# arangesh/TrackMPNN

Measured on AMD Instinct MI355X. Metric: graph_edges_per_sec_fwd_bwd, higher is better.
Workload: dtype f32; 1 GPU; C2 KITTI Car/RRC-shaped rolling windows: 7 frames, D_t~clip(Poisson(6),1,20), F=8 (2d), H=64, K=0, diff; 1 fwd per frame + 1 bwd per window; 16384 windows/GPU batched block-diagonally (64 distinct seeds tiled); windows_per_gpu=16384, rows_final=6762496, parallelism=sequence-dp1

## Files before the change

include/tmpnn.h:

```cpp
#ifndef TMPNN_H
#define TMPNN_H

#include <stddef.h>
#include <stdint.h>

#ifdef __cplusplus
extern "C" {
#endif

#define TMPNN_ABI_VERSION 4

#define TMPNN_OK 0
#define TMPNN_EINVAL (-1)
#define TMPNN_ELAUNCH (-2)
#define TMPNN_EWORKSPACE (-3)

typedef void* tmpnn_stream;
typedef void* tmpnn_event;

typedef struct tmpnn_seg_plan {
    int32_t T;
    int32_t I;
    int32_t nsplit;
    const int32_t* t_row;
// ... 111 lines not shown
                        float* d_msg, int ld_dmsg, float* d_h, int ld_dh,
                        const int32_t* add_src, const int32_t* add_dst, const float* add_msg, int ld_add,
                        float* dW_ih, float* dW_hh, float* db_ih, float* db_hh,
                        void* ws, size_t ws_bytes, tmpnn_stream stream);
int tmpnn_gru_bwd_fused_zero_state_available(int H, int IN, int xmode);
int tmpnn_gru_bwd_fused_zero_state(const int32_t* rows, int R, const int32_t* src, const int32_t* dst, int IN,
                                   const float* h, int ld_h, int H, const float* w_ih, const float* b_hn,
                                   const float* gates, size_t gate_plane, const float* d_hout, int ld_dhout,
                                   const float* dy, const float* w_head, float* d_msg, int ld_dmsg,
                                   float* dW_ih, float* db_ih, float* db_hh,
                                   void* ws, size_t ws_bytes, tmpnn_stream stream);

int tmpnn_gru_fwd_tiles(const tmpnn_edge_tiles* tiles, int R, const float* proj, int ld_proj, const float* h, int ld_h, int H,
                        const float* whh_t, const float* b_ih, const float* b_hh, float* h_out, int ld_out, float* gates,
                        size_t gate_plane, const float* w_head, float* logit_part, size_t part_stride, tmpnn_stream stream);

int tmpnn_rows_linear(const int32_t* rows, int R, const float* in, int ld_in, int H, const float* wt, int NOUT,
                      float* out, int ld_out, tmpnn_stream stream);

int tmpnn_transpose(const float* in, int rows, int cols, float* out, tmpnn_stream stream);

int tmpnn_input_bn_fwd(const float* xdet, int ld_x, int F, int nd, const int32_t* seg_ptr,
                       const int32_t* seg_cnt, const int32_t* seg_of_det ,
                       int S, int H, int training,
                       const float* w1, const float* b1, const float* gamma, const float* beta,
                       float* running_mean, float* running_var,
                       const float* w2, const float* b2,
                       float* y_save, float* mean, float* rstd, float* ws_a ,
                       const int32_t* out_row, float* h_new, int ld_h, tmpnn_stream stream);
size_t tmpnn_input_bn_bwd_ws(int nd, int S, int H, int F);
// ... 233 lines not shown
```

trackmpnn_amd/_lib.py:

```python
from __future__ import annotations

import ctypes as C

import torch
import os
import re
from typing import Dict, List, Optional

_HERE = os.path.dirname(os.path.abspath(__file__))
LIB_PATH = os.environ.get('TMPNN_LIB_PATH') or os.path.join(_HERE, 'lib', 'libtmpnn.so')
HEADER_PATH = os.path.join(os.path.dirname(_HERE), 'include', 'tmpnn.h')

ABI_VERSION = 4

c_int = C.c_int
c_void_p = C.c_void_p
c_size_t = C.c_size_t
c_float = C.c_float


class CSegPlan(C.Structure):
    _fields_ = [('T', C.c_int32), ('I', C.c_int32), ('nsplit', C.c_int32), ('t_row', c_void_p), ('items', c_void_p),
                ('rowptr2', c_void_p), ('inc2', c_void_p), ('ws', c_void_p), ('ws_floats', c_size_t)]

# ... 62 lines not shown
                              c_void_p, c_void_p, c_void_p, c_void_p, c_void_p, c_void_p, c_int, c_void_p]),
    'tmpnn_att_bwd_ws': (c_size_t, [c_int, c_int, c_int, c_int]),
    'tmpnn_att_index': (c_int, [_GP, c_void_p, c_void_p, c_void_p, c_void_p, c_void_p, c_void_p]),
    'tmpnn_att_bwd': (c_int, [_GP, c_void_p, c_void_p, c_void_p, c_int, c_int, c_int, c_void_p, c_void_p, c_void_p,
                              c_float, c_void_p, c_void_p, c_void_p, c_void_p, c_void_p, c_int, c_void_p, c_size_t,
                              c_void_p, c_int, c_void_p, c_void_p, c_void_p]),
    'tmpnn_att_bwd_heads': (c_int, [_GP, c_void_p, c_void_p, c_void_p, c_int, c_int, c_int, c_void_p, c_void_p,
                                    c_void_p, c_float, c_void_p, c_void_p, c_void_p, c_void_p, c_void_p, c_int, c_void_p,
                                    c_size_t, c_void_p, c_int, c_void_p, c_void_p, c_void_p]),
    'tmpnn_gru_fwd': (c_int, [c_void_p, c_int, c_int, c_void_p, c_void_p, c_void_p, c_int, c_int, c_int,
                              c_void_p, c_int, c_int, c_void_p, c_void_p, c_void_p, c_void_p,
                              c_void_p, c_int, c_void_p, c_size_t, c_void_p, c_void_p, c_size_t, c_void_p]),
    'tmpnn_gru_fwd_head_parts': (c_int, [c_int, c_int, c_int]),
    'tmpnn_gru_fwd_tiles': (c_int, [_TP, c_int, c_void_p, c_int, c_void_p, c_int, c_int, c_void_p, c_void_p, c_void_p,
                                    c_void_p, c_int, c_void_p, c_size_t, c_void_p, c_void_p, c_size_t, c_void_p]),
    'tmpnn_heads_finish': (c_int, [c_void_p, c_size_t, c_int, c_int, c_void_p, c_void_p, c_void_p, c_void_p, c_void_p, c_void_p]),
    'tmpnn_gru_bwd_data': (c_int, [c_void_p, c_int, c_int, c_void_p, c_int, c_int, c_void_p, c_void_p,
                                   c_void_p, c_size_t, c_void_p, c_int, c_void_p, c_void_p,
                                   c_void_p, c_int, c_void_p, c_int,
                                   c_void_p, c_void_p, c_void_p, c_int, c_void_p]),
    'tmpnn_gru_bwd_weights_ws': (c_size_t, [c_int, c_int, c_int]),
    'tmpnn_gru_bwd_weights': (c_int, [c_void_p, c_int, c_int, c_void_p, c_void_p, c_void_p, c_int, c_int, c_int,
                                      c_void_p, c_int, c_int, c_void_p, c_size_t, c_void_p, c_int, c_void_p, c_void_p,
                                      c_void_p, c_void_p, c_void_p, c_void_p, c_void_p, c_size_t, c_void_p]),
    'tmpnn_gru_bwd_fused_available': (c_int, [c_int, c_int, c_int]),
    'tmpnn_gru_bwd_fused_ws': (c_size_t, [c_int, c_int, c_int]),
    'tmpnn_gru_bwd_fused': (c_int, [c_void_p, c_int, c_int, c_void_p, c_void_p, c_void_p, c_int, c_int, c_int,
                                    c_void_p, c_int, c_int, c_void_p, c_void_p, c_void_p, c_size_t, c_void_p, c_int,
                                    c_void_p, c_void_p, c_void_p, c_int, c_void_p, c_int,
                                    c_void_p, c_void_p, c_void_p, c_int, c_void_p, c_void_p, c_void_p, c_void_p,
# ... 188 lines not shown
```

trackmpnn_amd/csrc/gru_fwd.hip:

```cpp
#include "gru_common.h"

namespace tmpnn {

template <int CT, int XMODE>
__global__ __launch_bounds__(256, 2) void k_gru_fwd(GruFwdArgs a) {
    const int wave = threadIdx.x >> 6, lane = threadIdx.x & 63;
    const int c = lane & 31, half = lane >> 5;
    const int r0 = (blockIdx.x * 4 + wave) * 32;
    if (r0 >= a.R) return;
    const int H = a.H, H3 = 3 * a.H;
    const int col0 = blockIdx.y * (32 * CT);
    const int li = min(r0 + c, a.R - 1);
    const int row = a.rows[li];

    f32x16 acc_r[CT], acc_z[CT], acc_in[CT], acc_hn[CT];
#pragma unroll
    for (int t = 0; t < CT; ++t)
#pragma unroll
        for (int i = 0; i < 16; ++i) { acc_r[t][i] = 0.f; acc_z[t][i] = 0.f; acc_in[t][i] = 0.f; acc_hn[t][i] = 0.f; }

    for (int kt = 0; kt < a.IN / 32; ++kt) {
        const int f0 = kt * 32 + half * 16;
        float av[16];
        load_x16<XMODE>(a, li, row, f0, av);
// ... 587 lines not shown
            if (half == 0 && r0 + c < a.R) a.logit_part[(size_t)cwb * a.part_stride + row] = p;
        }
        stage_store32(stg, c, half, lane, outv, a.h_out, a.ld_out, cw0, row, r0, a.R);
        if (a.gates) {
            stage_store32<true>(stg, c, half, lane, acc_r, a.gates, H, cw0, row, r0, a.R);
            stage_store32<true>(stg, c, half, lane, acc_z, a.gates + a.gate_plane, H, cw0, row, r0, a.R);
            stage_store32<true>(stg, c, half, lane, acc_in, a.gates + 2 * a.gate_plane, H, cw0, row, r0, a.R);
            stage_store32<true>(stg, c, half, lane, acc_hn, a.gates + 3 * a.gate_plane, H, cw0, row, r0, a.R);
        }
        if (!nvalid) break;
        r0 = nr0; li = nli; row = nrow;
    }
}

#define FT_MARK(i) do { } while (0)
struct FwdTiles { const int32_t* t_row; const int32_t* t_loc; const int32_t* t_dptr; const int32_t* t_dets; int T; };
static constexpr int TCAP = 24, TP_LD = 100;
static constexpr int TP_AREA = TCAP * TP_LD;

__device__ __forceinline__ uint32_t lds_addr_g(const void* p) {
    return (uint32_t)(uintptr_t)(const __attribute__((address_space(3))) char*)(const char*)p;
}
__device__ __forceinline__ void glds16_g(const void* gsrc, uint32_t lds_wave_base) {
    unsigned keep;
    lds_wave_base = __builtin_amdgcn_readfirstlane(lds_wave_base);
    asm volatile("s_mov_b32 %0, m0\n\ts_mov_b32 m0, %2\n\ts_nop 0\n\tglobal_load_lds_dwordx4 %1, off\n\ts_mov_b32 m0, %0"
                 : "=&s"(keep) : "v"(gsrc), "s"(lds_wave_base) : "memory");
}

struct TiledIdx { int row, loc, det, nd; };
__device__ __forceinline__ TiledIdx tiled_idx(const FwdTiles& tl, int R, int t, int c, int lane) {
// ... 25 lines not shown

template <int H>
__device__ __forceinline__ void tiled_stage_p2(const GruFwdArgs& a, const TiledIdx& x, int cw0, int lane, uint32_t area) {
    const int sub = lane >= 25 ? 1 : 0, rem = lane - 25 * sub;
    const int goff = (rem >> 3) * H + cw0 + 4 * (rem & 7);
    const bool lane_on = rem < 24 && lane < 49;
#pragma unroll 1
    for (int k = 0; 2 * k < x.nd; ++k) {
        const int d0 = __builtin_amdgcn_readlane(x.det, 2 * k), d1 = __builtin_amdgcn_readlane(x.det, min(2 * k + 1, 63));
        const int det = sub ? d1 : d0;
        if (lane_on && 2 * k + sub < x.nd) glds16_g(a.msg + (size_t)det * a.ld_msg + goff, area + 800u * k);
    }
}

#define FT_STAGE_P tiled_stage_p2
template <int H, int WPB>
__global__ __launch_bounds__(WPB * 64) void k_gru_fwd_split_tiled(GruFwdArgs a, FwdTiles tl) {
    extern __shared__ float lds[];
    constexpr int H3 = 3 * H, KP = H + 8, NKB = H / 16, CW = H / 32, NQ4 = H / 8;
    uint16_t* sW = reinterpret_cast<uint16_t*>(lds);
    for (int i = threadIdx.x; i < H * H3 / 4; i += WPB * 64) {
        const int k = i / (H3 / 4), j0 = (i % (H3 / 4)) * 4;
        const float4 w = *reinterpret_cast<const float4*>(a.whh_t + (size_t)k * H3 + j0);
        const float wv[4] = {w.x, w.y, w.z, w.w};
#pragma unroll
        for (int e = 0; e < 4; ++e) {
            uint16_t q1, q2, q3;
            split1(wv[e], q1, q2, q3);
            sW[(0 * H3 + j0 + e) * KP + k] = q1;
            sW[(1 * H3 + j0 + e) * KP + k] = q2;
            sW[(2 * H3 + j0 + e) * KP + k] = q3;
        }
    }
    float* area_base = reinterpret_cast<float*>(sW + 3 * H3 * KP);
    int* next_item = reinterpret_cast<int*>(area_base + WPB * TP_AREA);
    float* sBias = reinterpret_cast<float*>(next_item + 4);
    for (int i = threadIdx.x; i < H; i += WPB * 64) {
        sBias[i] = a.b_ih[i] + a.b_hh[i];
        sBias[H + i] = a.b_ih[H + i] + a.b_hh[H + i];
        sBias[2 * H + i] = a.b_ih[2 * H + i];
        sBias[3 * H + i] = a.b_hh[2 * H + i];
        sBias[4 * H + i] = a.logit_part ? a.w_head[i] : 0.f;
    }
    if (threadIdx.x == 0) *next_item = 0;
    __syncthreads();
    const int wave = threadIdx.x >> 6, lane = threadIdx.x & 63;
    const int c = lane & 31, half = lane >> 5;
    {
        const int grp = __builtin_amdgcn_readfirstlane(wave) >> 2;
// ... 5 lines not shown
    const int per_block = (items_total + gridDim.x - 1) / gridDim.x;
    const int item_lo = blockIdx.x * per_block;
    const int item_hi = min(items_total, item_lo + per_block);

    int item = 0;
    if (lane == 0) item = atomicAdd(next_item, 1);
    item = __builtin_amdgcn_readfirstlane(item) + item_lo;
    if (item >= item_hi) return;
    int cw0 = (item % CW) * 32;
    int t = item / CW;
    TiledIdx ix = tiled_idx(tl, a.R, t, c, lane);
    float* stg = area_base + wave * TP_AREA;
    const uint32_t area = lds_addr_g(stg);
    if (ix.nd <= TCAP) FT_STAGE_P<H>(a, ix, cw0, lane, area);
    float4 raw[NQ4];
    {
        const float4* xr = reinterpret_cast<const float4*>(a.h + (size_t)ix.row * a.ld_h + (H / 2) * half);
#pragma unroll
        for (int i = 0; i < NQ4; ++i) raw[i] = xr[i];
    }

    for (;;) {
        int nitem = 0;
        if (lane == 0) nitem = atomicAdd(next_item, 1);
        nitem = __builtin_amdgcn_readfirstlane(nitem) + item_lo;
        const bool nvalid = nitem < item_hi;
        const int ncw0 = (nitem % CW) * 32;
        const int nt = nvalid ? nitem / CW : t;
        const int r0 = 32 * t;
        const int row = ix.row;
        const bool staged = ix.nd <= TCAP;
        Split8 b[NKB];
#pragma unroll
        for (int kb = 0; kb < NKB; ++kb) b[kb] = split8(raw[2 * kb], raw[2 * kb + 1]);
        const TiledIdx nix = tiled_idx(tl, a.R, nt, c, lane);
        if (nvalid) {
            const float4* xr = reinterpret_cast<const float4*>(a.h + (size_t)nix.row * a.ld_h + (H / 2) * half);
#pragma unroll
            for (int i = 0; i < NQ4; ++i) raw[i] = xr[i];
        }
        f32x16 acc_r, acc_z, acc_hn, acc_in;
#pragma unroll
        for (int i = 0; i < 16; ++i) { acc_r[i] = 0.f; acc_z[i] = 0.f; acc_hn[i] = 0.f; }
        {
            const uint16_t* wp0 = sW + (cw0 + c) * KP + (H / 2) * half;
#pragma unroll
            for (int kb = 0; kb < NKB; ++kb) {
                const uint16_t* wp = wp0 + 8 * kb;
#pragma unroll
                for (int g = 0; g < 3; ++g) {
                    const uint4 w1 = *reinterpret_cast<const uint4*>(wp + (g * H) * KP);
                    const uint4 w2 = *reinterpret_cast<const uint4*>(wp + (H3 + g * H) * KP);
                    const uint4 w3 = *reinterpret_cast<const uint4*>(wp + (2 * H3 + g * H) * KP);
                    if (g == 0) acc_r = mfma_x6(w1, w2, w3, b[kb], acc_r);
                    else if (g == 1) acc_z = mfma_x6(w1, w2, w3, b[kb], acc_z);
                    else acc_hn = mfma_x6(w1, w2, w3, b[kb], acc_hn);
                }
            }
        }
        if (staged) {
            if (nvalid) {
                if constexpr (NQ4 == 8) asm volatile("s_waitcnt vmcnt(8)" ::: "memory");
                else asm volatile("s_waitcnt vmcnt(4)" ::: "memory");
            } else {
                asm volatile("s_waitcnt vmcnt(0)" ::: "memory");
            }
        }
        float4 hp4[4];
#pragma unroll
        for (int q = 0; q < 4; ++q)
            hp4[q] = *reinterpret_cast<const float4*>(a.h + (size_t)row * a.ld_h + cw0 + 8 * q + 4 * half);
        f32x16 outv;
        {
            float4 gs[4], gd[4], hs[4], hd[4];
            const int ls = ix.loc & 0xFFFF, ld_ = ix.loc >> 16;
            const int sdet = __shfl(ix.det, ls, 64), ddet = __shfl(ix.det, ld_, 64);
            const float* ps0 = a.msg + (size_t)sdet * a.ld_msg + cw0 + 4 * half;
            const float* pd0 = a.msg + (size_t)ddet * a.ld_msg + cw0 + 4 * half;
            if (staged) {
                const float* ls0 = stg + ls * TP_LD + 4 * half;
                const float* ld0 = stg + ld_ * TP_LD + 4 * half;
#pragma unroll
                for (int q = 0; q < 4; ++q) gs[q] = *reinterpret_cast<const float4*>(ls0 + 8 * q);
#pragma unroll
                for (int q = 0; q < 4; ++q) gd[q] = *reinterpret_cast<const float4*>(ld0 + 8 * q);
#pragma unroll
// ... 71 lines not shown
            float p = 0.f;
#pragma unroll
            for (int q = 0; q < 4; ++q) {
                const float4 w = *reinterpret_cast<const float4*>(sBias + 4 * H + cw0 + 8 * q + 4 * half);
                p += outv[4 * q] * w.x + outv[4 * q + 1] * w.y + outv[4 * q + 2] * w.z + outv[4 * q + 3] * w.w;
            }
            p += __shfl_xor(p, 32);
            if (half == 0 && r0 + c < a.R) a.logit_part[(size_t)(cw0 / 32) * a.part_stride + row] = p;
        }
        asm volatile("s_waitcnt lgkmcnt(0)" ::: "memory");
        stage_store32(stg, c, half, lane, outv, a.h_out, a.ld_out, cw0, row, r0, a.R);
        if (a.gates) {
            stage_store32<true>(stg, c, half, lane, acc_r, a.gates, H, cw0, row, r0, a.R);
            stage_store32<true>(stg, c, half, lane, acc_z, a.gates + a.gate_plane, H, cw0, row, r0, a.R);
            stage_store32<true>(stg, c, half, lane, acc_in, a.gates + 2 * a.gate_plane, H, cw0, row, r0, a.R);
            stage_store32<true>(stg, c, half, lane, acc_hn, a.gates + 3 * a.gate_plane, H, cw0, row, r0, a.R);
        }
        if (!nvalid) break;
        cw0 = ncw0; t = nt; ix = nix;
        if (ix.nd <= TCAP) FT_STAGE_P<H>(a, ix, cw0, lane, area);
    }
}


static constexpr int T16_CAP = 12;
static constexpr int T16_AREA = T16_CAP * TP_LD;

__device__ __forceinline__ f32x4 mfma16_x6(const uint4& a1, const uint4& a2, const uint4& a3, const Split8& b, f32x4 c) {
    c = __builtin_amdgcn_mfma_f32_16x16x32_bf16(__builtin_bit_cast(bf16x8, a3), __builtin_bit_cast(bf16x8, b.p1), c, 0, 0, 0);
    c = __builtin_amdgcn_mfma_f32_16x16x32_bf16(__builtin_bit_cast(bf16x8, a1), __builtin_bit_cast(bf16x8, b.p3), c, 0, 0, 0);
    c = __builtin_amdgcn_mfma_f32_16x16x32_bf16(__builtin_bit_cast(bf16x8, a2), __builtin_bit_cast(bf16x8, b.p2), c, 0, 0, 0);
// ... 538 lines not shown
            hipLaunchKernelGGL((k_gru_fwd_split_t16<32, 16>), pgrid, dim3(1024), shm16, st, a, tl);
        }
        return check_launch("gru_fwd_split_t16");
    }
    const size_t shm = (size_t)3 * 3 * H * (H + 8) * 2 + sizeof(float) * ((size_t)8 * TP_AREA + 4 + 5 * H);
    if (H == 64) {
        TM_SHM_ONCE((k_gru_fwd_split_tiled<64, 8>), shm);
        hipLaunchKernelGGL((k_gru_fwd_split_tiled<64, 8>), pgrid, dim3(512), shm, st, a, tl);
    } else {
        TM_SHM_ONCE((k_gru_fwd_split_tiled<32, 8>), shm);
        hipLaunchKernelGGL((k_gru_fwd_split_tiled<32, 8>), pgrid, dim3(512), shm, st, a, tl);
    }
    return check_launch("gru_fwd_split_tiled");
}

int tmpnn_rows_linear(const int32_t* rows, int R, const float* in, int ld_in, int H, const float* wt, int NOUT,
                      float* out, int ld_out, tmpnn_stream stream) {
    TM_REQUIRE((H == 32 || H == 64) && (NOUT == 3 * H), "rows_linear: only [H<=64] x [3H] projections (H=%d NOUT=%d)", H, NOUT);
    if (R == 0) return TMPNN_OK;
    TM_REQUIRE(R > 0 && rows && in && wt && out, "rows_linear: null pointer");
    TM_REQUIRE(ld_in >= H && (ld_in & 3) == 0 && aligned16(in) && aligned16(wt) && ld_out >= NOUT && (ld_out & 3) == 0 &&
                   aligned16(out),
               "rows_linear: rows must be 16-byte aligned");
    const int ntiles = ceil_div(R, 256);
    dim3 grid(ntiles < 256 ? ntiles : 256), block(512);
    hipStream_t st = as_stream(stream);
    if (split_enabled()) return launch_rows_gemm(rows, R, in, ld_in, H, wt, NOUT, 0, NOUT, out, ld_out, nullptr, 0, st);
    const size_t shm = sizeof(float) * ((size_t)H * NOUT + 8 * 32 * STG_LD);
    if (H == 64) {
        TM_SHM_ONCE((k_rows_gemm_lds<64, 6>), shm);
// ... 10 lines not shown
```

trackmpnn_amd/functional.py:

```python
from __future__ import annotations

import contextlib
import ctypes
import os
from dataclasses import dataclass
from typing import Dict, List, Optional, Sequence, Tuple

import torch

from . import _lib
from .graph import CallPlan, dense_seg_plan, edge_tiles, win_plan

ATT_DROPOUT_P = 0.5
INPLACE_GRADS = os.environ.get('TMPNN_INPLACE_GRADS', '0') == '1'
FUSED_BWD = os.environ.get('TMPNN_FUSED_BWD', '1') == '1'
ZERO_STATE_BWD = os.environ.get('TMPNN_BWD_ZERO_STATE', '1') != '0'
WIDE_OVERLAP = os.environ.get('TMPNN_WIDE_OVERLAP', '0') == '1' and os.environ.get('TMPNN_KEEP_VARIANTS', '0') == '1'
ATT_KMAX = 8
_SPLIT = os.environ.get('TMPNN_SPLIT', '1')[:1] != '0'

_VARIANTS = os.environ.get('TMPNN_KEEP_VARIANTS', '0') == '1'


def _variant(name: str, default: str) -> str:
    return os.environ.get(name, default) if _VARIANTS else default


WIDE_DW = _variant('TMPNN_WIDE_DW', '1') == '1'
WIDE_DET = _variant('TMPNN_WIDE_DET', '1') == '1'
WIDE = _variant('TMPNN_WIDE', '1') != '0' and _SPLIT
WIDE_TILED = _variant('TMPNN_WIDE_TILED', '1') != '0'
# ... 192 lines not shown

    opts = dict(dtype=torch.float32, device=dev)
    h_cat = None
    if h_in is not None and N_old > 0 and n > 0 and h_in.is_contiguous():
        st_ = h_in.untyped_storage()
        if h_spare >= n and st_.nbytes() >= 4 * (h_in.storage_offset() + N * GH):
            h_cat = torch.empty(0, **opts).set_(st_, h_in.storage_offset(), (N, GH), (GH, 1))
    if h_cat is None:
        if h_in is not None and n == 0:
            h_cat = h_in
        else:
            h_cat = torch.empty((N, GH), **opts)
            if N_old > 0:
                h_cat[:N_old].copy_(h_in)
    saved = dict(n=n)
    if n > 0:
        h_cat[N_old:].zero_()
        nd = int(plan.new_det_row.numel())
        S = plan.S
        if training and plan.min_seg_cnt <= 1:
            raise ValueError('Expected more than 1 value per channel when training, got input size '
                             f'[1, {H}]')
        tf_all = nd > 0 and all(_input_tf(plan, H, F) for _, F in spec.groups)
        if tf_all:
            xsrc, xrows = _f32c(x.detach()), plan.new_det_local
            if xrows.dtype != torch.int64 or not xrows.is_contiguous():
                xrows = xrows.long().contiguous()
            xdet = None
        else:
            xdet = _f32c(x.detach().index_select(0, plan.new_det_local)) if nd > 0 else torch.empty((0, spec.F_total), **opts)
            xsrc, xrows = xdet, None
        ws_a = torch.empty((max(nd, 1), H), **opts)
# ... 32 lines not shown
        if save:
            saved.update(xdet=xsrc, xrows=xrows, y_save=y_saves, mean=means, rstd=rstds)

    spare = max(int(reserve_rows), 0)
    if spare > 0:
        buf = torch.empty(((N + spare) * GH,), **opts)
        h_out = torch.empty(0, **opts).set_(buf.untyped_storage(), 0, (N, GH), (GH, 1))
    else:
        h_out = torch.empty((N, GH), **opts)
    gates = torch.empty((G, 4, N, H), **opts) if save else None
    es_all = torch.empty((G, max(Dn, 1), H), **opts)
    alphas: List[Optional[List[torch.Tensor]]] = []
    att_saved = []
    xmode = 2 if spec.msg_type == 'concat' else 1
    plane = N * H
    lib = _lib.load()
    use_proj = spec.msg_type == 'diff' and H <= 64 and g.src_pos is not None and Dn > 0
    use_proj_cat = (CONCAT_PROJ and spec.msg_type == 'concat' and H <= 64 and FWD_TILED and g.src_pos is not None
                    and Dn > 0 and E > 0)
    use_wide = (WIDE and spec.msg_type == 'diff' and H >= 128 and bool(lib.tmpnn_wide_supported(H, H))
                and g.src_pos is not None and Dn > 0 and E > 0)
    if use_wide and H % 256 == 0 and K == 0:
        dense_seg_plan(g)
    if WIN_SEGSUM and H == 64 and E > 0:
        win_plan(g)
    wide_preps = []
    zero_from = N_old if n > 0 else N
    cw = min(lib.tmpnn_gru_fwd_head_parts(H, H if use_proj_cat else spec.IN_e, 3 if (use_proj or use_proj_cat) else xmode),
             lib.tmpnn_gru_fwd_head_parts(H, H, 0))
    parts = torch.empty((G * cw, N), **opts) if cw > 0 else None
    w_node, w_edge = P['output_transform_node.weight'], P['output_transform_edge.weight']
# ... 33 lines not shown
            proj = torch.empty((2 * Dn, 3 * H), **opts)
            _lib.call('tmpnn_rows_linear', g.det_row.data_ptr(), Dn, hg, GH, H, e_wih_t.data_ptr(), 3 * H,
                      proj.data_ptr(), 3 * H, st)
            w2n = _cached(('negt', e_wih_t.data_ptr(), H), (e_wih_t,), lambda: e_wih_t[H:].neg().contiguous())
            _lib.call('tmpnn_rows_linear', g.det_row.data_ptr(), Dn, hg, GH, H, w2n.data_ptr(), 3 * H,
                      proj.data_ptr() + 4 * Dn * 3 * H, 3 * H, st)
            _lib.call('tmpnn_gru_fwd_tiles', edge_tiles(g, FWD_TILE_ROWS, dst_offset=Dn).cref(), E, proj.data_ptr(), 3 * H, hg, GH,
                      H, e_whh_t.data_ptr(), P[f + 'edge_gru.bias_ih'].data_ptr(), P[f + 'edge_gru.bias_hh'].data_ptr(),
                      og, GH, gp, plane, we_g, part_g, N, st)
        elif use_proj:
            proj = torch.empty((Dn, 3 * H), **opts)
            _lib.call('tmpnn_rows_linear', g.det_row.data_ptr(), Dn, hg, GH, H, e_wih_t.data_ptr(), 3 * H,
                      proj.data_ptr(), 3 * H, st)
            if FWD_TILED and E > 0:
                recompute = RECOMPUTE_GATES and save
                _lib.call('tmpnn_gru_fwd_tiles', edge_tiles(g, FWD_TILE_ROWS).cref(), E, proj.data_ptr(), 3 * H, hg, GH, H,
                          e_whh_t.data_ptr(), P[f + 'edge_gru.bias_ih'].data_ptr(), P[f + 'edge_gru.bias_hh'].data_ptr(),
                          og, GH, None if recompute else gp, plane, we_g, part_g, N, st)
                if recompute:
                    saved.setdefault('proj', {})[gi] = (proj, e_whh_t)
            else:
                _lib.call('tmpnn_gru_fwd', g.edge_row.data_ptr(), E, 3, g.src_pos.data_ptr(), g.dst_pos.data_ptr(),
                          proj.data_ptr(), 3 * H, 0, H, hg, GH, H, None, e_whh_t.data_ptr(),
                          P[f + 'edge_gru.bias_ih'].data_ptr(), P[f + 'edge_gru.bias_hh'].data_ptr(),
                          og, GH, gp, plane, we_g, part_g, N, st)
        else:
            _lib.call('tmpnn_gru_fwd', g.edge_row.data_ptr(), E, xmode, g.src.data_ptr(), g.dst.data_ptr(),
                      None, 0, 0, spec.IN_e, hg, GH, H,
                      e_wih_t.data_ptr(), e_whh_t.data_ptr(),
                      P[f + 'edge_gru.bias_ih'].data_ptr(), P[f + 'edge_gru.bias_hh'].data_ptr(),
                      og, GH, gp, plane, we_g, part_g, N, st)
        es = es_all[gi]
        if K == 0:
# ... 129 lines not shown
        if use_fused_bwd:
            _lib.call('tmpnn_gru_bwd_fused', g.det_row.data_ptr(), Dn, 0, None, None, es.data_ptr(), H, 1, H,
                      hg, GH, H, P[f + 'node_gru.weight_ih'].data_ptr(), P[f + 'node_gru.weight_hh'].data_ptr(),
                      gp, plane, dog, GH, dyp, wn, dmsg.data_ptr(), IN_e, dhg, GH, None, None, None, 0,
                      grads[f + 'node_gru.weight_ih'].data_ptr(), grads[f + 'node_gru.weight_hh'].data_ptr(),
                      grads[f + 'node_gru.bias_ih'].data_ptr(), grads[f + 'node_gru.bias_hh'].data_ptr(),
                      ws_w.data_ptr(), ws_w.numel() * 4, st)
            if saved.get('proj') and gi in saved['proj']:
                proj_s, whh_t_s = saved['proj'][gi]
                h_scr = _wide_workspace(4 * N * GH, dev, slot=2)
                _lib.call('tmpnn_gru_fwd_tiles', edge_tiles(g, FWD_TILE_ROWS).cref(), E, proj_s.data_ptr(), 3 * H, hg, GH, H,
                          whh_t_s.data_ptr(), P[f + 'edge_gru.bias_ih'].data_ptr(), P[f + 'edge_gru.bias_hh'].data_ptr(),
                          h_scr.data_ptr() + 4 * gi * H, GH, gp, plane, None, None, 0, st)
            b_hn = P[f + 'edge_gru.bias_hh'].data_ptr() + 4 * 2 * H
            E_old = E - (n - int(plan.new_det_row.numel())) if n > 0 else E
            zs = (ZERO_STATE_BWD and n > 0 and K == 0 and xmode == 1 and 0 <= E_old < E and b_hn % 16 == 0
                  and not (saved.get('proj') and gi in saved['proj'])
                  and lib.tmpnn_gru_bwd_fused_zero_state_available(H, IN_e, xmode))
            E_full = E_old if zs else E
            if E_full > 0:
                _lib.call('tmpnn_gru_bwd_fused', g.edge_row.data_ptr(), E_full, xmode, g.src.data_ptr(), g.dst.data_ptr(),
                          None, 0, 0, IN_e, hg, GH, H,
                          P[f + 'edge_gru.weight_ih'].data_ptr(), P[f + 'edge_gru.weight_hh'].data_ptr(),
                          gp, plane, dog, GH, dyp, we, dmsg.data_ptr(), IN_e, dhg, GH,
                          g.src.data_ptr() if fuse else None, g.dst.data_ptr() if fuse else None,
                          dmsg.data_ptr() if fuse else None, IN_e,
                          grads[f + 'edge_gru.weight_ih'].data_ptr(), grads[f + 'edge_gru.weight_hh'].data_ptr(),
                          grads[f + 'edge_gru.bias_ih'].data_ptr(), grads[f + 'edge_gru.bias_hh'].data_ptr(),
                          ws_w.data_ptr(), ws_w.numel() * 4, st)
            if zs:
                _lib.call('tmpnn_gru_bwd_fused_zero_state', g.edge_row.data_ptr() + 4 * E_old, E - E_old,
                          g.src.data_ptr() + 4 * E_old, g.dst.data_ptr() + 4 * E_old, IN_e, hg, GH, H,
                          P[f + 'edge_gru.weight_ih'].data_ptr(), b_hn, gp, plane, dog, GH, dyp, we,
# ... 199 lines not shown
```

trackmpnn_amd/graph.py:

```python
from __future__ import annotations

import ctypes as C
from dataclasses import dataclass, field
from typing import List, Optional, Sequence, Tuple

import numpy as np
import torch

from . import _lib


@dataclass
class FrameGraph:
    N: int
    E: int
    Dn: int
    src: torch.Tensor
    dst: torch.Tensor
    edge_row: torch.Tensor
    det_row: torch.Tensor
    rowptr: torch.Tensor
    inc: torch.Tensor
    is_edge: torch.Tensor
    pos: torch.Tensor
# ... 70 lines not shown
    t_row: torch.Tensor
    t_loc: torch.Tensor
    t_dptr: torch.Tensor
    t_dets: torch.Tensor
    max_dets: int = 0
    _c: Optional[_lib.CEdgeTiles] = field(default=None, repr=False, compare=False)

    def cref(self):
        if self._c is None:
            self._c = _lib.CEdgeTiles(self.T, self.rows_per_tile, self.t_row.data_ptr(), self.t_loc.data_ptr(),
                                      self.t_dptr.data_ptr(), self.t_dets.data_ptr())
        return C.byref(self._c)


def build_edge_tiles(graph: FrameGraph, rows_per_tile: int = 128, src_group: int = 8, dst_group: int = 16,
                     stats: bool = False, order: str = 'blocks', dst_offset: int = 0) -> EdgeTiles:
    if graph.src_pos is None or graph.dst_pos is None:
        raise ValueError('build_edge_tiles: the graph carries no src_pos / dst_pos')
    dev = graph.device
    E, R = graph.E, int(rows_per_tile)
    T = (E + R - 1) // R
    i32 = lambda t: t.to(torch.int32).contiguous()
    if T == 0:
        z = torch.zeros(0, dtype=torch.int32, device=dev)
        return EdgeTiles(0, R, z, z.clone(), torch.zeros(1, dtype=torch.int32, device=dev), z.clone())
    s, d = graph.src_pos.long(), graph.dst_pos.long()
    ns = graph.Dn // src_group + 1
    if order == 'rows':
        so, do, ro = s, d, graph.edge_row.long()
    else:
        key = (((d // dst_group) * ns + s // src_group) * src_group + s % src_group) * dst_group + d % dst_group
        perm = torch.argsort(key)
        so, do, ro = s[perm], d[perm], graph.edge_row.long()[perm]
    pad = T * R - E
    if pad:
        so = torch.cat([so, so[-1:].expand(pad)])
        do = torch.cat([do, do[-1:].expand(pad)])
        ro = torch.cat([ro, torch.full((pad,), -1, dtype=torch.long, device=dev)])
    both = torch.cat([so.view(T, R), do.view(T, R) + int(dst_offset)], 1)
    vals, perm = both.sort(1)
    first = torch.ones_like(vals, dtype=torch.bool)
    first[:, 1:] = vals[:, 1:] != vals[:, :-1]
    rank = first.long().cumsum(1) - 1
    local = torch.empty_like(rank)
    local.scatter_(1, perm, rank)
    cnt = rank[:, -1] + 1
    dptr = torch.zeros(T + 1, dtype=torch.long, device=dev)
    dptr[1:] = cnt.cumsum(0)
    loc = local[:, :R] | (local[:, R:] << 16)
    tiles = EdgeTiles(T, R, i32(ro), i32(loc.reshape(-1)), i32(dptr), i32(vals[first]))
    if stats:
        tiles.max_dets = int(cnt.max())
    return tiles


def edge_tiles(graph: FrameGraph, rows_per_tile: int = 128, dst_offset: int = 0) -> EdgeTiles:
    cache = graph.__dict__.setdefault('_tiles', {})
    key = rows_per_tile if not dst_offset else (rows_per_tile, int(dst_offset))
    t = cache.get(key)
    if t is None:
        runs = 1
        if graph.E > 1:
            if graph.src_pos.is_cuda and torch.cuda.is_current_stream_capturing():
                raise RuntimeError('edge_tiles: the tile list of this graph is not built yet and building it reads one '
                                   'count back to the host, which a stream capture cannot do -- run one eager call on the '
                                   'graph (CapturedWindow does) before capturing')
            runs = 1 + int((graph.src_pos[1:] != graph.src_pos[:-1]).sum())
        blocks = graph.E / runs >= rows_per_tile / 2
        od = 'blocks' if blocks else 'rows'
        if rows_per_tile == 128:
            t = build_edge_tiles(graph, 128, 8, 16, order=od, dst_offset=dst_offset)
        elif rows_per_tile == 16:
            t = build_edge_tiles(graph, 16, 4, 4, order=od, dst_offset=dst_offset)
        else:
            t = build_edge_tiles(graph, rows_per_tile, 4, 8, order=od, dst_offset=dst_offset)
        cache[key] = t
    return t


class SegPlan:

    def __init__(self, T, I, nsplit, t_row, items, rowptr2, inc2, ws):
        self.T, self.I, self.nsplit = int(T), int(I), int(nsplit)
        self.t_row, self.items, self.rowptr2, self.inc2, self.ws = t_row, items, rowptr2, inc2, ws
        self.c = _lib.CSegPlan(self.T, self.I, self.nsplit, t_row.data_ptr(), items.data_ptr(), rowptr2.data_ptr(),
                               inc2.data_ptr(), ws.data_ptr(), ws.numel())


SEG_ITEM_TILES = 13

# ... 646 lines not shown
```

Baseline: 682.3 million graph-edges/s.

## Add zero-state GRU forward kernel for new-edge rows and skip their state zeroing

Splits the edge GRU forward into two launches: the old edges go through the normal tiled kernel, and the new edges, whose hidden state is known to be zero, use a templated zero-state variant. That variant skips loading W_hh into LDS, the hidden-state reads and the recurrent matmul, and uses a higher occupancy launch bound. It can also skip writing the hn gate plane and skip zeroing h_cat for new rows when the zero-state backward consumes them. The cost is an extra launch, an extra set of cached edge tiles per range, and more conditions that must agree between forward and backward.

Measured after the change: 704.3 million graph-edges/s, median of 6. +3.2%, better.

```diff
diff --git a/include/tmpnn.h b/include/tmpnn.h
--- a/include/tmpnn.h
+++ b/include/tmpnn.h
@@ -149,6 +149,11 @@
 int tmpnn_gru_fwd_tiles(const tmpnn_edge_tiles* tiles, int R, const float* proj, int ld_proj, const float* h, int ld_h, int H,
                         const float* whh_t, const float* b_ih, const float* b_hh, float* h_out, int ld_out, float* gates,
                         size_t gate_plane, const float* w_head, float* logit_part, size_t part_stride, tmpnn_stream stream);
+int tmpnn_gru_fwd_tiles_zero_state_available(int H, int xmode);
+int tmpnn_gru_fwd_tiles_zero_state(const tmpnn_edge_tiles* tiles, int R, const float* proj, int ld_proj, int H,
+                                   const float* b_ih, const float* b_hh, float* h_out, int ld_out, float* gates,
+                                   size_t gate_plane, int write_hn, const float* w_head, float* logit_part, size_t part_stride,
+                                   tmpnn_stream stream);
 
 int tmpnn_rows_linear(const int32_t* rows, int R, const float* in, int ld_in, int H, const float* wt, int NOUT,
                       float* out, int ld_out, tmpnn_stream stream);
diff --git a/trackmpnn_amd/_lib.py b/trackmpnn_amd/_lib.py
--- a/trackmpnn_amd/_lib.py
+++ b/trackmpnn_amd/_lib.py
@@ -100,6 +100,9 @@
     'tmpnn_gru_fwd_head_parts': (c_int, [c_int, c_int, c_int]),
     'tmpnn_gru_fwd_tiles': (c_int, [_TP, c_int, c_void_p, c_int, c_void_p, c_int, c_int, c_void_p, c_void_p, c_void_p,
                                     c_void_p, c_int, c_void_p, c_size_t, c_void_p, c_void_p, c_size_t, c_void_p]),
+    'tmpnn_gru_fwd_tiles_zero_state_available': (c_int, [c_int, c_int]),
+    'tmpnn_gru_fwd_tiles_zero_state': (c_int, [_TP, c_int, c_void_p, c_int, c_int, c_void_p, c_void_p, c_void_p, c_int,
+                                               c_void_p, c_size_t, c_int, c_void_p, c_void_p, c_size_t, c_void_p]),
     'tmpnn_heads_finish': (c_int, [c_void_p, c_size_t, c_int, c_int, c_void_p, c_void_p, c_void_p, c_void_p, c_void_p, c_void_p]),
     'tmpnn_gru_bwd_data': (c_int, [c_void_p, c_int, c_int, c_void_p, c_int, c_int, c_void_p, c_void_p,
                                    c_void_p, c_size_t, c_void_p, c_int, c_void_p, c_void_p,
diff --git a/trackmpnn_amd/csrc/gru_fwd.hip b/trackmpnn_amd/csrc/gru_fwd.hip
--- a/trackmpnn_amd/csrc/gru_fwd.hip
+++ b/trackmpnn_amd/csrc/gru_fwd.hip
@@ -625,7 +625,7 @@
 }
 
 #define FT_MARK(i) do { } while (0)
-struct FwdTiles { const int32_t* t_row; const int32_t* t_loc; const int32_t* t_dptr; const int32_t* t_dets; int T; };
+struct FwdTiles { const int32_t* t_row; const int32_t* t_loc; const int32_t* t_dptr; const int32_t* t_dets; int T; int zs_hn; };
 static constexpr int TCAP = 24, TP_LD = 100;
 static constexpr int TP_AREA = TCAP * TP_LD;
 
@@ -681,11 +681,12 @@
 }
 
 #define FT_STAGE_P tiled_stage_p2
-template <int H, int WPB>
-__global__ __launch_bounds__(WPB * 64) void k_gru_fwd_split_tiled(GruFwdArgs a, FwdTiles tl) {
+template <int H, int WPB, bool ZS = false>
+__global__ __launch_bounds__(WPB * 64, ZS ? 3 : 1) void k_gru_fwd_split_tiled(GruFwdArgs a, FwdTiles tl) {
     extern __shared__ float lds[];
     constexpr int H3 = 3 * H, KP = H + 8, NKB = H / 16, CW = H / 32, NQ4 = H / 8;
     uint16_t* sW = reinterpret_cast<uint16_t*>(lds);
+    if constexpr (!ZS)
     for (int i = threadIdx.x; i < H * H3 / 4; i += WPB * 64) {
         const int k = i / (H3 / 4), j0 = (i % (H3 / 4)) * 4;
         const float4 w = *reinterpret_cast<const float4*>(a.whh_t + (size_t)k * H3 + j0);
@@ -699,7 +700,7 @@
             sW[(2 * H3 + j0 + e) * KP + k] = q3;
         }
     }
-    float* area_base = reinterpret_cast<float*>(sW + 3 * H3 * KP);
+    float* area_base = reinterpret_cast<float*>(sW + (ZS ? 0 : 3 * H3 * KP));
     int* next_item = reinterpret_cast<int*>(area_base + WPB * TP_AREA);
     float* sBias = reinterpret_cast<float*>(next_item + 4);
     for (int i = threadIdx.x; i < H; i += WPB * 64) {
@@ -735,7 +736,7 @@
     const uint32_t area = lds_addr_g(stg);
     if (ix.nd <= TCAP) FT_STAGE_P<H>(a, ix, cw0, lane, area);
     float4 raw[NQ4];
-    {
+    if constexpr (!ZS) {
         const float4* xr = reinterpret_cast<const float4*>(a.h + (size_t)ix.row * a.ld_h + (H / 2) * half);
 #pragma unroll
         for (int i = 0; i < NQ4; ++i) raw[i] = xr[i];
@@ -752,18 +753,22 @@
         const int row = ix.row;
         const bool staged = ix.nd <= TCAP;
         Split8 b[NKB];
-#pragma unroll
-        for (int kb = 0; kb < NKB; ++kb) b[kb] = split8(raw[2 * kb], raw[2 * kb + 1]);
+        if constexpr (!ZS) {
+#pragma unroll
+            for (int kb = 0; kb < NKB; ++kb) b[kb] = split8(raw[2 * kb], raw[2 * kb + 1]);
+        }
         const TiledIdx nix = tiled_idx(tl, a.R, nt, c, lane);
-        if (nvalid) {
-            const float4* xr = reinterpret_cast<const float4*>(a.h + (size_t)nix.row * a.ld_h + (H / 2) * half);
-#pragma unroll
-            for (int i = 0; i < NQ4; ++i) raw[i] = xr[i];
+        if constexpr (!ZS) {
+            if (nvalid) {
+                const float4* xr = reinterpret_cast<const float4*>(a.h + (size_t)nix.row * a.ld_h + (H / 2) * half);
+#pragma unroll
+                for (int i = 0; i < NQ4; ++i) raw[i] = xr[i];
+            }
         }
         f32x16 acc_r, acc_z, acc_hn, acc_in;
 #pragma unroll
         for (int i = 0; i < 16; ++i) { acc_r[i] = 0.f; acc_z[i] = 0.f; acc_hn[i] = 0.f; }
-        {
+        if constexpr (!ZS) {
             const uint16_t* wp0 = sW + (cw0 + c) * KP + (H / 2) * half;
 #pragma unroll
             for (int kb = 0; kb < NKB; ++kb) {
@@ -780,7 +785,7 @@
             }
         }
         if (staged) {
-            if (nvalid) {
+            if (!ZS && nvalid) {
                 if constexpr (NQ4 == 8) asm volatile("s_waitcnt vmcnt(8)" ::: "memory");
                 else asm volatile("s_waitcnt vmcnt(4)" ::: "memory");
             } else {
@@ -788,9 +793,14 @@
             }
         }
         float4 hp4[4];
-#pragma unroll
-        for (int q = 0; q < 4; ++q)
-            hp4[q] = *reinterpret_cast<const float4*>(a.h + (size_t)row * a.ld_h + cw0 + 8 * q + 4 * half);
+        if constexpr (ZS) {
+#pragma unroll
+            for (int q = 0; q < 4; ++q) hp4[q] = make_float4(0.f, 0.f, 0.f, 0.f);
+        } else {
+#pragma unroll
+            for (int q = 0; q < 4; ++q)
+                hp4[q] = *reinterpret_cast<const float4*>(a.h + (size_t)row * a.ld_h + cw0 + 8 * q + 4 * half);
+        }
         f32x16 outv;
         {
             float4 gs[4], gd[4], hs[4], hd[4];
@@ -892,7 +902,7 @@
             stage_store32<true>(stg, c, half, lane, acc_r, a.gates, H, cw0, row, r0, a.R);
             stage_store32<true>(stg, c, half, lane, acc_z, a.gates + a.gate_plane, H, cw0, row, r0, a.R);
             stage_store32<true>(stg, c, half, lane, acc_in, a.gates + 2 * a.gate_plane, H, cw0, row, r0, a.R);
-            stage_store32<true>(stg, c, half, lane, acc_hn, a.gates + 3 * a.gate_plane, H, cw0, row, r0, a.R);
+            if (!ZS || tl.zs_hn) stage_store32<true>(stg, c, half, lane, acc_hn, a.gates + 3 * a.gate_plane, H, cw0, row, r0, a.R);
         }
         if (!nvalid) break;
         cw0 = ncw0; t = nt; ix = nix;
@@ -1461,6 +1471,44 @@
     return check_launch("gru_fwd_split_tiled");
 }
 
+int tmpnn_gru_fwd_tiles_zero_state_available(int H, int xmode) { return (H == 32 || H == 64) && xmode == 3 && split_enabled(); }
+
+int tmpnn_gru_fwd_tiles_zero_state(const tmpnn_edge_tiles* tiles, int R, const float* proj, int ld_proj, int H,
+                                   const float* b_ih, const float* b_hh, float* h_out, int ld_out, float* gates,
+                                   size_t gate_plane, int write_hn, const float* w_head, float* logit_part, size_t part_stride,
+                                   tmpnn_stream stream) {
+    TM_REQUIRE(tmpnn_gru_fwd_tiles_zero_state_available(H, 3), "gru_fwd_tiles_zero_state: H=%d (H in {32, 64}, TMPNN_SPLIT on)", H);
+    TM_REQUIRE(R >= 0, "gru_fwd_tiles_zero_state: R=%d", R);
+    if (R == 0) return TMPNN_OK;
+    TM_REQUIRE(tiles != nullptr, "gru_fwd_tiles_zero_state: tiles is null");
+    TM_REQUIRE(tiles->rows_per_tile == 32 && tiles->T > 0 && (long)tiles->T * 32 >= R && (long)(tiles->T - 1) * 32 < R &&
+                   tiles->t_row && tiles->t_loc && tiles->t_dptr && tiles->t_dets,
+               "gru_fwd_tiles_zero_state: tile list (T=%d, rows_per_tile=%d) does not cover R=%d rows in 32-row tiles", tiles->T,
+               tiles->rows_per_tile, R);
+    TM_REQUIRE(proj && b_ih && b_hh && h_out, "gru_fwd_tiles_zero_state: null pointer");
+    TM_REQUIRE(ld_proj >= 3 * H && (ld_proj & 3) == 0 && aligned16(proj) && ld_out >= H && aligned16(h_out) && (ld_out & 3) == 0 &&
+                   aligned16(b_ih) && aligned16(b_hh) &&
+                   (gates == nullptr || (aligned16(gates) && (gate_plane & 3) == 0 && gate_plane >= (size_t)H)),
+               "gru_fwd_tiles_zero_state: layout (16-byte alignment, leading dimensions)");
+    TM_REQUIRE(logit_part == nullptr || (w_head != nullptr && aligned16(w_head)),
+               "gru_fwd_tiles_zero_state: fused head needs a 16-byte aligned w_head");
+    GruFwdArgs a{nullptr, R, nullptr, nullptr, proj, ld_proj, H, 0, nullptr, 0, H, nullptr, nullptr, b_ih, b_hh, h_out, ld_out,
+                 gates, gate_plane, w_head, logit_part, part_stride};
+    FwdTiles tl{tiles->t_row, tiles->t_loc, tiles->t_dptr, tiles->t_dets, tiles->T, write_hn ? 1 : 0};
+    hipStream_t st = as_stream(stream);
+    const int ntiles = ceil_div(R, (H == 64) ? 96 : 128);
+    dim3 pgrid(ntiles < 768 ? ntiles : 768);
+    const size_t shm = sizeof(float) * ((size_t)4 * TP_AREA + 4 + 5 * H);
+    if (H == 64) {
+        TM_SHM_ONCE((k_gru_fwd_split_tiled<64, 4, true>), shm);
+        hipLaunchKernelGGL((k_gru_fwd_split_tiled<64, 4, true>), pgrid, dim3(256), shm, st, a, tl);
+    } else {
+        TM_SHM_ONCE((k_gru_fwd_split_tiled<32, 4, true>), shm);
+        hipLaunchKernelGGL((k_gru_fwd_split_tiled<32, 4, true>), pgrid, dim3(256), shm, st, a, tl);
+    }
+    return check_launch("gru_fwd_split_tiled_zs");
+}
+
 int tmpnn_rows_linear(const int32_t* rows, int R, const float* in, int ld_in, int H, const float* wt, int NOUT,
                       float* out, int ld_out, tmpnn_stream stream) {
     TM_REQUIRE((H == 32 || H == 64) && (NOUT == 3 * H), "rows_linear: only [H<=64] x [3H] projections (H=%d NOUT=%d)", H, NOUT);
diff --git a/trackmpnn_amd/functional.py b/trackmpnn_amd/functional.py
--- a/trackmpnn_amd/functional.py
+++ b/trackmpnn_amd/functional.py
@@ -15,6 +15,7 @@
 INPLACE_GRADS = os.environ.get('TMPNN_INPLACE_GRADS', '0') == '1'
 FUSED_BWD = os.environ.get('TMPNN_FUSED_BWD', '1') == '1'
 ZERO_STATE_BWD = os.environ.get('TMPNN_BWD_ZERO_STATE', '1') != '0'
+ZERO_STATE_FWD = os.environ.get('TMPNN_FWD_ZERO_STATE', '1') != '0'
 WIDE_OVERLAP = os.environ.get('TMPNN_WIDE_OVERLAP', '0') == '1' and os.environ.get('TMPNN_KEEP_VARIANTS', '0') == '1'
 ATT_KMAX = 8
 _SPLIT = os.environ.get('TMPNN_SPLIT', '1')[:1] != '0'
@@ -237,8 +238,20 @@
             if N_old > 0:
                 h_cat[:N_old].copy_(h_in)
     saved = dict(n=n)
+    lib = _lib.load()
+    E_old = E - (n - int(plan.new_det_row.numel())) if n > 0 else E
+    zs_fwd = (ZERO_STATE_FWD and n > 0 and K == 0 and spec.msg_type == 'diff' and H == 64 and g.src_pos is not None
+              and Dn > 0 and FWD_TILED and FWD_TILE_ROWS == 32 and 0 <= E_old < E and not RECOMPUTE_GATES
+              and all((P[f'factor_grus.{gi}.edge_gru.bias_hh'].data_ptr() + 4 * 2 * H) % 16 == 0 for gi in range(G))
+              and bool(lib.tmpnn_gru_fwd_tiles_zero_state_available(H, 3)))
+    zs_bwd = (zs_fwd and save and ZERO_STATE_BWD and FUSED_BWD and bool(lib.tmpnn_gru_bwd_fused_available(H, H, 0))
+              and bool(lib.tmpnn_gru_bwd_fused_available(H, spec.IN_e, 1))
+              and bool(lib.tmpnn_gru_bwd_fused_zero_state_available(H, spec.IN_e, 1)))
+    if zs_fwd and save:
+        saved['zs_bwd'] = zs_bwd
     if n > 0:
-        h_cat[N_old:].zero_()
+        if not (zs_fwd and (zs_bwd or not save)):
+            h_cat[N_old:].zero_()
         nd = int(plan.new_det_row.numel())
         S = plan.S
         if training and plan.min_seg_cnt <= 1:
@@ -301,7 +314,6 @@
     att_saved = []
     xmode = 2 if spec.msg_type == 'concat' else 1
     plane = N * H
-    lib = _lib.load()
     use_proj = spec.msg_type == 'diff' and H <= 64 and g.src_pos is not None and Dn > 0
     use_proj_cat = (CONCAT_PROJ and spec.msg_type == 'concat' and H <= 64 and FWD_TILED and g.src_pos is not None
                     and Dn > 0 and E > 0)
@@ -365,9 +377,17 @@
                       proj.data_ptr(), 3 * H, st)
             if FWD_TILED and E > 0:
                 recompute = RECOMPUTE_GATES and save
-                _lib.call('tmpnn_gru_fwd_tiles', edge_tiles(g, FWD_TILE_ROWS).cref(), E, proj.data_ptr(), 3 * H, hg, GH, H,
-                          e_whh_t.data_ptr(), P[f + 'edge_gru.bias_ih'].data_ptr(), P[f + 'edge_gru.bias_hh'].data_ptr(),
-                          og, GH, None if recompute else gp, plane, we_g, part_g, N, st)
+                E_full = E_old if zs_fwd else E
+                if E_full > 0:
+                    tiles = edge_tiles(g, FWD_TILE_ROWS, e1=E_full)
+                    _lib.call('tmpnn_gru_fwd_tiles', tiles.cref(), E_full, proj.data_ptr(), 3 * H, hg, GH, H,
+                              e_whh_t.data_ptr(), P[f + 'edge_gru.bias_ih'].data_ptr(), P[f + 'edge_gru.bias_hh'].data_ptr(),
+                              og, GH, None if recompute else gp, plane, we_g, part_g, N, st)
+                if zs_fwd:
+                    _lib.call('tmpnn_gru_fwd_tiles_zero_state', edge_tiles(g, FWD_TILE_ROWS, e0=E_old).cref(), E - E_old,
+                              proj.data_ptr(), 3 * H, H, P[f + 'edge_gru.bias_ih'].data_ptr(),
+                              P[f + 'edge_gru.bias_hh'].data_ptr(), og, GH, gp, plane, int(save and not zs_bwd), we_g,
+                              part_g, N, st)
                 if recompute:
                     saved.setdefault('proj', {})[gi] = (proj, e_whh_t)
             else:
@@ -527,9 +547,12 @@
                           h_scr.data_ptr() + 4 * gi * H, GH, gp, plane, None, None, 0, st)
             b_hn = P[f + 'edge_gru.bias_hh'].data_ptr() + 4 * 2 * H
             E_old = E - (n - int(plan.new_det_row.numel())) if n > 0 else E
-            zs = (ZERO_STATE_BWD and n > 0 and K == 0 and xmode == 1 and 0 <= E_old < E and b_hn % 16 == 0
-                  and not (saved.get('proj') and gi in saved['proj'])
-                  and lib.tmpnn_gru_bwd_fused_zero_state_available(H, IN_e, xmode))
+            if 'zs_bwd' in saved:
+                zs = saved['zs_bwd']
+            else:
+                zs = (ZERO_STATE_BWD and n > 0 and K == 0 and xmode == 1 and 0 <= E_old < E and b_hn % 16 == 0
+                      and not (saved.get('proj') and gi in saved['proj'])
+                      and lib.tmpnn_gru_bwd_fused_zero_state_available(H, IN_e, xmode))
             E_full = E_old if zs else E
             if E_full > 0:
                 _lib.call('tmpnn_gru_bwd_fused', g.edge_row.data_ptr(), E_full, xmode, g.src.data_ptr(), g.dst.data_ptr(),
diff --git a/trackmpnn_amd/graph.py b/trackmpnn_amd/graph.py
--- a/trackmpnn_amd/graph.py
+++ b/trackmpnn_amd/graph.py
@@ -108,24 +108,29 @@
 
 
 def build_edge_tiles(graph: FrameGraph, rows_per_tile: int = 128, src_group: int = 8, dst_group: int = 16,
-                     stats: bool = False, order: str = 'blocks', dst_offset: int = 0) -> EdgeTiles:
+                     stats: bool = False, order: str = 'blocks', dst_offset: int = 0,
+                     e0: int = 0, e1: Optional[int] = None) -> EdgeTiles:
     if graph.src_pos is None or graph.dst_pos is None:
         raise ValueError('build_edge_tiles: the graph carries no src_pos / dst_pos')
     dev = graph.device
-    E, R = graph.E, int(rows_per_tile)
+    e1 = graph.E if e1 is None else int(e1)
+    e0 = int(e0)
+    if not 0 <= e0 <= e1 <= graph.E:
+        raise ValueError(f'build_edge_tiles: edge range [{e0}, {e1}) outside [0, {graph.E})')
+    E, R = e1 - e0, int(rows_per_tile)
     T = (E + R - 1) // R
     i32 = lambda t: t.to(torch.int32).contiguous()
     if T == 0:
         z = torch.zeros(0, dtype=torch.int32, device=dev)
         return EdgeTiles(0, R, z, z.clone(), torch.zeros(1, dtype=torch.int32, device=dev), z.clone())
-    s, d = graph.src_pos.long(), graph.dst_pos.long()
+    s, d = graph.src_pos[e0:e1].long(), graph.dst_pos[e0:e1].long()
     ns = graph.Dn // src_group + 1
     if order == 'rows':
-        so, do, ro = s, d, graph.edge_row.long()
+        so, do, ro = s, d, graph.edge_row[e0:e1].long()
     else:
         key = (((d // dst_group) * ns + s // src_group) * src_group + s % src_group) * dst_group + d % dst_group
         perm = torch.argsort(key)
-        so, do, ro = s[perm], d[perm], graph.edge_row.long()[perm]
+        so, do, ro = s[perm], d[perm], graph.edge_row[e0:e1].long()[perm]
     pad = T * R - E
     if pad:
         so = torch.cat([so, so[-1:].expand(pad)])
@@ -148,9 +153,13 @@
     return tiles
 
 
-def edge_tiles(graph: FrameGraph, rows_per_tile: int = 128, dst_offset: int = 0) -> EdgeTiles:
+def edge_tiles(graph: FrameGraph, rows_per_tile: int = 128, dst_offset: int = 0, e0: int = 0,
+               e1: Optional[int] = None) -> EdgeTiles:
     cache = graph.__dict__.setdefault('_tiles', {})
+    e1 = graph.E if e1 is None else int(e1)
     key = rows_per_tile if not dst_offset else (rows_per_tile, int(dst_offset))
+    if (int(e0), e1) != (0, graph.E):
+        key = (key, int(e0), e1)
     t = cache.get(key)
     if t is None:
         runs = 1
@@ -162,12 +171,13 @@
             runs = 1 + int((graph.src_pos[1:] != graph.src_pos[:-1]).sum())
         blocks = graph.E / runs >= rows_per_tile / 2
         od = 'blocks' if blocks else 'rows'
+        rng = dict(order=od, dst_offset=dst_offset, e0=e0, e1=e1)
         if rows_per_tile == 128:
-            t = build_edge_tiles(graph, 128, 8, 16, order=od, dst_offset=dst_offset)
+            t = build_edge_tiles(graph, 128, 8, 16, **rng)
         elif rows_per_tile == 16:
-            t = build_edge_tiles(graph, 16, 4, 4, order=od, dst_offset=dst_offset)
+            t = build_edge_tiles(graph, 16, 4, 4, **rng)
         else:
-            t = build_edge_tiles(graph, rows_per_tile, 4, 8, order=od, dst_offset=dst_offset)
+            t = build_edge_tiles(graph, rows_per_tile, 4, 8, **rng)
         cache[key] = t
     return t
 
```
